# MisEty/X-SLAM

Hardware: AMD Instinct MI355X
Metric: fps XKinectFusion 512^3 TSDF 640x480 CSFD @1/2/4/8 GPU; HBM GB/s on integrate (higher is better)
Workload: dtype f32 (complex<f32> CSFD)

## Files before the change

### include/xslam_amd.h

```cpp
#ifndef XSLAM_AMD_H
#define XSLAM_AMD_H
#include <stddef.h>
#include <stdint.h>

#ifdef __cplusplus
extern "C" {
#endif

const char *xs_last_error(void);

unsigned xs_const_div_prepare(float c);
unsigned xs_const_div_state(float c);
int xs_const_div_enable(int on);
int xs_abi_version(void);

int xs_init_volume(float *value, int *weight, float *grad, size_t step_bytes, const int *res, int z0, int z1, void *stream);

int xs_scale_depth(const uint16_t *depth, size_t depth_step, int rows, int cols, float *scaled, size_t scaled_step, void *stream);
int xs_scale_depth_max(const uint16_t *depth, size_t depth_step, int rows, int cols, float *scaled, size_t scaled_step,
                       float *max_dev, void *stream);
size_t xs_depth_tiles_bytes(int rows, int cols);
int xs_scale_depth_tiles(const uint16_t *depth, size_t depth_step, int rows, int cols, float *scaled, size_t scaled_step,
                         float *max_dev, void *tiles_dev, void *stream);
int xs_depth_tiles(const float *scaled, size_t scaled_step, int rows, int cols, void *tiles_dev, void *stream);
// ... 25 lines not shown
int xs_integrate_list_covers(int rows, int cols, const float *intr4, const int *res, float voxel_size, const float *Rv2c18_list,
                             const float *tv2c6_list, float slack_scale, const float *Rv2c18, const float *tv2c6);
size_t xs_integrate_workspace_bytes(const int *res, int nz);

typedef struct xs_integrate_opts {
    unsigned struct_bytes;
    unsigned flags;
    const void *depth_tiles;
    void *signmap;
    void *start_event, *stop_event;
} xs_integrate_opts;
int xs_integrate_scaled_ex2(const float *depth_scaled, size_t scaled_step, int rows, int cols, const float *intr4, int max_weight,
                            const int *res, float voxel_size, const float *Rv2c18, const float *tv2c6, float tranc_dist, float *value,
                            int *weight, float *grad, size_t vol_step, float threshold, int z0, int z1,
                            unsigned long long *updated_dev, const float *depth_max_dev, void *workspace, const xs_integrate_opts *opts, void *stream);
int xs_integrate_classify_ex(int rows, int cols, const float *intr4, const int *res, float voxel_size, const float *Rv2c18, const float *tv2c6,
                             float tranc_dist, int z0, int z1, const float *depth_max_dev, void *workspace, float slack_scale,
                             const xs_integrate_opts *opts, void *stream);
typedef struct xs_raycast_opts {
    unsigned struct_bytes;
    int signmap_shift;
    const void *signmap;
    float signmap_tranc_dist;
    float *pyr_vmap1, *pyr_nmap1;
    size_t pyr_step1;
    float *pyr_vmap2, *pyr_nmap2;
    size_t pyr_step2;
    void *completion_event;
    int *steps_dev;
    int pyramid_built;
} xs_raycast_opts;
int xs_raycast_ex(const float *intr4, const float *Rc2v18, const float *tc2v6, const float *Rv2w18, const float *tv2w6,
                  float tranc_dist, const int *res, float voxel_size, const float *value, const float *grad, size_t vol_step,
                  float *vmap, float *nmap, size_t map_step, int rows, int cols, unsigned long long *hits_dev, float *workspace,
                  xs_raycast_opts *opts, void *stream);
int xs_raycast_slab_ex(const float *intr4, const float *Rc2v18, const float *tc2v6, const float *Rv2w18, const float *tv2w6,
                       float tranc_dist, const int *res, float voxel_size, const float *value, const float *grad, size_t vol_step,
                       int zs0, int zs1, int z0, int z1, float *vmap, float *nmap, size_t map_step, int rows, int cols, int *keys_dev,
                       const xs_raycast_opts *opts, void *stream);
int xs_resize_pyramid_ex(const float *vmap0, const float *nmap0, size_t in_step, int rows0, int cols0, float *vmap1, float *nmap1,
                         size_t mid_step, float *vmap2, float *nmap2, size_t out_step, void *completion_event, void *stream);

size_t xs_tsdf_reduce_workspace_bytes(void);
int xs_tsdf_reduce_workspace_init(void *workspace, void *stream);
int xs_compute_local_tsdf_hessian(const float *depth_scaled, size_t scaled_step, int rows, int cols, const float *intr4,
                                  const int *res, float voxel_size, const float *Rv2c36, const float *tv2c12, float tranc_dist,
                                  const float *gt, float *real_out, float *grad_out, float *hess_out, int *count_out, int z0, int z1,
                                  void *workspace, double *out4_dev, void *stream);
int xs_compute_local_tsdf_loss(const float *depth_scaled, size_t scaled_step, int rows, int cols, const float *intr4, const int *res,
                               float voxel_size, const float *Rv2c9, const float *tv2c3, float tranc_dist, const float *gt,
                               float *real_out, int *count_out, int z0, int z1, void *workspace, double *out2_dev, void *stream);

int xs_bilateral_filter(const uint16_t *src, size_t src_step, int rows, int cols, float *dst, size_t dst_step, void *stream);
int xs_pyr_down(const float *src, size_t src_step, int src_rows, int src_cols, float *dst, size_t dst_step, void *stream);
int xs_create_vmap(const float *intr4, const float *depth, size_t depth_step, int rows, int cols, float *vmap, size_t vmap_step,
                   void *stream);
int xs_create_nmap(const float *vmap, float *nmap, size_t map_step, int rows, int cols, void *stream);
int xs_create_vnmaps(int levels, const float *intr4s, const float *const *depths, const size_t *depth_steps, int rows0, int cols0,
                     float *const *vmaps, float *const *nmaps, const size_t *map_steps, void *stream);
int xs_create_vnmaps_real(int levels, const float *intr4s, const float *const *depths, const size_t *depth_steps, int rows0, int cols0,
                          float *const *vmaps, float *const *nmaps, const size_t *map_steps, float *const *vreal, float *const *nreal,
                          const size_t *real_steps, void *stream);
int xs_resize_vmap(const float *in, size_t in_step, int src_rows, int src_cols, float *out, size_t out_step, void *stream);
int xs_resize_nmap(const float *in, size_t in_step, int src_rows, int src_cols, float *out, size_t out_step, void *stream);
int xs_resize_pyramid(const float *vmap0, const float *nmap0, size_t in_step, int rows0, int cols0, float *vmap1, float *nmap1,
                      size_t mid_step, float *vmap2, float *nmap2, size_t out_step, void *stream);

int xs_raycast(const float *intr4, const float *Rc2v18, const float *tc2v6, const float *Rv2w18, const float *tv2w6,
               float tranc_dist, const int *res, float voxel_size, const float *value, const float *grad, size_t vol_step,
               float *vmap, float *nmap, size_t map_step, int rows, int cols, unsigned long long *hits_dev, float *workspace,
               void *stream);

int xs_raycast_signmap_shift(const float *intr4, float voxel_size, float tranc_dist);
size_t xs_signmap_bytes(const int *res, int shift);
int xs_signmap_reset(void *signmap, const int *res, int shift, float tranc_dist, void *stream);
int xs_signmap_rebuild(void *signmap, const int *res, int shift, float tranc_dist, const float *value, size_t vol_step, void *stream);
int xs_signmap_rebuild_slab(void *signmap, const int *res, int shift, float tranc_dist, const float *value, size_t vol_step, int zs0, int zs1,
                            void *stream);


int xs_raycast_slab(const float *intr4, const float *Rc2v18, const float *tc2v6, const float *Rv2w18, const float *tv2w6,
                    float tranc_dist, const int *res, float voxel_size, const float *value, const float *grad, size_t vol_step,
                    int zs0, int zs1, int z0, int z1, float *vmap, float *nmap, size_t map_step, int rows, int cols, int *keys_dev,
                    void *stream);
int xs_raycast_compose_mask(const int *own_keys_dev, const int *min_keys_dev, float *vmap, float *nmap, size_t map_step, int rows,
                            int cols, void *stream);
int xs_raycast_compose_finish(const int *min_keys_dev, float *vmap, float *nmap, size_t map_step, int rows, int cols,
                              unsigned long long *hits_dev, void *stream);
size_t xs_raycast_compose_entry_bytes(void);
int xs_raycast_compose_pack(const int *own_keys_dev, const int *min_keys_dev, const float *vmap, const float *nmap, size_t map_step, int rows, int cols,
                            void *entries_dev, int *count_dev, void *stream);
int xs_raycast_compose_scatter(const void *entries_dev, long n, float *vmap, float *nmap, size_t map_step, int rows, int cols, void *stream);

int xs_tsdf_gauss_newton_terms(const float *depth_scaled, size_t scaled_step, int rows, int cols, const float *intr4, const int *res,
                               float voxel_size, const float *Rv2c108, const float *tv2c36, float tranc_dist, const float *gt, int z0, int z1,
                               void *workspace, double *out29_dev, void *stream);
typedef struct xs_gn_opts {
    unsigned struct_bytes;
    unsigned mailbox_seq;
    const void *pose_mailbox;
    double *publish_host;
    unsigned long long publish_seq;
} xs_gn_opts;
int xs_tsdf_gauss_newton_terms_ex(const float *depth_scaled, size_t scaled_step, int rows, int cols, const float *intr4, const int *res,
                                  float voxel_size, const float *Rv2c108, const float *tv2c36, float tranc_dist, const float *gt, int z0, int z1,
                                  void *workspace, double *out29_dev, const xs_gn_opts *opts, void *stream);
// ... 258 lines not shown
```

### x-slam_amd/capi.py

```python
import ctypes as C
import os

import numpy as np

_HERE = os.path.dirname(os.path.abspath(__file__))
LIB_PATH = os.path.join(_HERE, "libxslam_hip.so")

_vp = C.c_void_p
_sz = C.c_size_t
_f32p = C.POINTER(C.c_float)
_i32p = C.POINTER(C.c_int)
_f64p = C.POINTER(C.c_double)


class XsError(RuntimeError):
    pass


def _load():
    if not os.path.exists(LIB_PATH):
        raise ImportError(
            f"{LIB_PATH} not found: build the HIP extension first (python -c 'import __graft_entry__ as g; g.build()' "
            "or make -C x-slam_amd/csrc).  There is no CPU fallback.")
    return C.CDLL(LIB_PATH)
# ... 72 lines not shown
    "xs_frontier_label_bytes": (_sz, [_i32p]),
    "xs_frontier_workspace_bytes": (_sz, [_i32p, C.c_int]),
    "xs_frontier_mask": (C.c_int, [_vp, _i32p, _vp, _vp]),
    "xs_frontier_label": (C.c_int, [_vp, _i32p, C.c_int, _vp, _vp, _i32p, _vp]),
    "xs_frontier_clusters": (C.c_int, [_vp, _vp, _i32p, C.c_int, _vp, _vp, C.POINTER(C.c_uint), _vp, _vp]),
    "xs_frontier_expand": (C.c_int, [_vp, _i32p, _vp, _vp]),
    "xs_integrate_scaled_ex2": (C.c_int, [_vp, _sz, C.c_int, C.c_int, _f32p, C.c_int, _i32p, C.c_float, _f32p, _f32p, C.c_float, _vp, _vp, _vp,
                                         _sz, C.c_float, C.c_int, C.c_int, _vp, _vp, _vp, C.POINTER(IntegrateOpts), _vp]),
    "xs_integrate_classify_ex": (C.c_int, [C.c_int, C.c_int, _f32p, _i32p, C.c_float, _f32p, _f32p, C.c_float, C.c_int, C.c_int, _vp, _vp,
                                           C.c_float, C.POINTER(IntegrateOpts), _vp]),
    "xs_raycast_ex": (C.c_int, [_f32p, _f32p, _f32p, _f32p, _f32p, C.c_float, _i32p, C.c_float, _vp, _vp, _sz, _vp, _vp, _sz,
                                C.c_int, C.c_int, _vp, _vp, C.POINTER(RaycastOpts), _vp]),
    "xs_raycast_slab_ex": (C.c_int, [_f32p, _f32p, _f32p, _f32p, _f32p, C.c_float, _i32p, C.c_float, _vp, _vp, _sz, C.c_int, C.c_int,
                                     C.c_int, C.c_int, _vp, _vp, _sz, C.c_int, C.c_int, _vp, C.POINTER(RaycastOpts), _vp]),
    "xs_resize_pyramid_ex": (C.c_int, [_vp, _vp, _sz, C.c_int, C.c_int, _vp, _vp, _sz, _vp, _vp, _sz, _vp, _vp]),
    "xs_last_error": (C.c_char_p, []),
    "xs_abi_version": (C.c_int, []),
    "xs_init_volume": (C.c_int, [_vp, _vp, _vp, _sz, _i32p, C.c_int, C.c_int, _vp]),
    "xs_scale_depth": (C.c_int, [_vp, _sz, C.c_int, C.c_int, _vp, _sz, _vp]),
    "xs_integrate_tsdf_volume": (C.c_int, [_vp, _sz, C.c_int, C.c_int, _f32p, C.c_int, _i32p, C.c_float, _f32p, _f32p, C.c_float,
                                           _vp, _vp, _vp, _sz, _vp, _sz, C.c_float, C.c_int, C.c_int, _vp, _vp]),
    "xs_integrate_scaled": (C.c_int, [_vp, _sz, C.c_int, C.c_int, _f32p, C.c_int, _i32p, C.c_float, _f32p, _f32p, C.c_float,
                                      _vp, _vp, _vp, _sz, C.c_float, C.c_int, C.c_int, _vp, _vp, _vp, _vp]),
    "xs_integrate_scaled_ex": (C.c_int, [_vp, _sz, C.c_int, C.c_int, _f32p, C.c_int, _i32p, C.c_float, _f32p, _f32p, C.c_float, _vp, _vp, _vp,
                                        _sz, C.c_float, C.c_int, C.c_int, _vp, _vp, _vp, C.c_uint, _vp]),
    "xs_integrate_workspace_clear": (C.c_int, [_vp, _vp]),
    "xs_integrate_fold_counts": (C.c_int, [_vp, _vp, _vp]),
    "xs_integrate_classify": (C.c_int, [C.c_int, C.c_int, _f32p, _i32p, C.c_float, _f32p, _f32p, C.c_float, C.c_int, C.c_int, _vp, _vp,
                                        C.c_float, C.c_uint, _vp]),
    "xs_integrate_list_covers": (C.c_int, [C.c_int, C.c_int, _f32p, _i32p, C.c_float, _f32p, _f32p, C.c_float, _f32p, _f32p]),
    "xs_integrate_workspace_bytes": (_sz, [_i32p, C.c_int]),
    "xs_scale_depth_max": (C.c_int, [_vp, _sz, C.c_int, C.c_int, _vp, _sz, _vp, _vp]),
    "xs_scale_depth_tiles": (C.c_int, [_vp, _sz, C.c_int, C.c_int, _vp, _sz, _vp, _vp, _vp]),
    "xs_depth_tiles": (C.c_int, [_vp, _sz, C.c_int, C.c_int, _vp, _vp]),
    "xs_depth_tiles_bytes": (_sz, [C.c_int, C.c_int]),
    "xs_tsdf_reduce_workspace_bytes": (_sz, []),
    "xs_tsdf_band_segs_bytes": (_sz, [_i32p, C.c_int, C.c_int]),
    "xs_tsdf_band_build": (C.c_int, [_vp, _i32p, C.c_int, C.c_int, C.POINTER(BandIndex), _vp]),
    "xs_tsdf_band_workspace_bytes": (_sz, [C.c_int]),
    "xs_tsdf_gauss_newton_terms_band": (C.c_int, [C.c_int, C.POINTER(_vp), _sz, C.c_int, C.c_int, _f32p, C.c_float, _f32p, _f32p, C.c_float,
                                                  C.POINTER(BandIndex), _vp, _vp, _vp]),
    "xs_tsdf_pose_hessian_workspace_bytes": (_sz, [C.c_int]),
    "xs_tsdf_pose_hessian_band": (C.c_int, [C.c_int, C.POINTER(_vp), _sz, C.c_int, C.c_int, _f32p, C.c_float, _f32p, _f32p, C.c_float,
                                            C.POINTER(BandIndex), _vp, _vp, _vp]),
    "xs_tsdf_score_poses_workspace_bytes": (_sz, [C.c_int]),
    "xs_tsdf_score_poses_band": (C.c_int, [C.c_int, _vp, _sz, C.c_int, C.c_int, _f32p, C.c_float, _f32p, _f32p, C.c_float, C.POINTER(BandIndex), _vp,
                                           _vp, _vp]),
    "xs_tsdf_reduce_workspace_init": (C.c_int, [_vp, _vp]),
    "xs_compute_local_tsdf_hessian": (C.c_int, [_vp, _sz, C.c_int, C.c_int, _f32p, _i32p, C.c_float, _f32p, _f32p, C.c_float, _vp,
                                                _vp, _vp, _vp, _vp, C.c_int, C.c_int, _vp, _vp, _vp]),
    "xs_compute_local_tsdf_loss": (C.c_int, [_vp, _sz, C.c_int, C.c_int, _f32p, _i32p, C.c_float, _f32p, _f32p, C.c_float, _vp,
                                             _vp, _vp, C.c_int, C.c_int, _vp, _vp, _vp]),
    "xs_bilateral_filter": (C.c_int, [_vp, _sz, C.c_int, C.c_int, _vp, _sz, _vp]),
    "xs_pyr_down": (C.c_int, [_vp, _sz, C.c_int, C.c_int, _vp, _sz, _vp]),
    "xs_create_vmap": (C.c_int, [_f32p, _vp, _sz, C.c_int, C.c_int, _vp, _sz, _vp]),
    "xs_create_nmap": (C.c_int, [_vp, _vp, _sz, C.c_int, C.c_int, _vp]),
    "xs_create_vnmaps": (C.c_int, [C.c_int, _f32p, C.POINTER(_vp), C.POINTER(_sz), C.c_int, C.c_int, C.POINTER(_vp), C.POINTER(_vp),
                                   C.POINTER(_sz), _vp]),
    "xs_create_vnmaps_real": (C.c_int, [C.c_int, _f32p, C.POINTER(_vp), C.POINTER(_sz), C.c_int, C.c_int, C.POINTER(_vp), C.POINTER(_vp),
                                        C.POINTER(_sz), C.POINTER(_vp), C.POINTER(_vp), C.POINTER(_sz), _vp]),
    "xs_resize_vmap": (C.c_int, [_vp, _sz, C.c_int, C.c_int, _vp, _sz, _vp]),
    "xs_resize_nmap": (C.c_int, [_vp, _sz, C.c_int, C.c_int, _vp, _sz, _vp]),
    "xs_raycast": (C.c_int, [_f32p, _f32p, _f32p, _f32p, _f32p, C.c_float, _i32p, C.c_float, _vp, _vp, _sz, _vp, _vp, _sz,
                             C.c_int, C.c_int, _vp, _vp, _vp]),
    "xs_raycast_slab": (C.c_int, [_f32p, _f32p, _f32p, _f32p, _f32p, C.c_float, _i32p, C.c_float, _vp, _vp, _sz, C.c_int, C.c_int,
                                  C.c_int, C.c_int, _vp, _vp, _sz, C.c_int, C.c_int, _vp, _vp]),
    "xs_raycast_compose_mask": (C.c_int, [_vp, _vp, _vp, _vp, _sz, C.c_int, C.c_int, _vp]),
    "xs_raycast_compose_finish": (C.c_int, [_vp, _vp, _vp, _sz, C.c_int, C.c_int, _vp, _vp]),
    "xs_raycast_compose_entry_bytes": (_sz, []),
    "xs_raycast_compose_pack": (C.c_int, [_vp, _vp, _vp, _vp, _sz, C.c_int, C.c_int, _vp, _vp, _vp]),
    "xs_raycast_compose_scatter": (C.c_int, [_vp, C.c_long, _vp, _vp, _sz, C.c_int, C.c_int, _vp]),
    "xs_resize_pyramid": (C.c_int, [_vp, _vp, _sz, C.c_int, C.c_int, _vp, _vp, _sz, _vp, _vp, _sz, _vp]),
    "xs_tsdf_gauss_newton_terms": (C.c_int, [_vp, _sz, C.c_int, C.c_int, _f32p, _i32p, C.c_float, _f32p, _f32p, C.c_float, _vp, C.c_int,
                                             C.c_int, _vp, _vp, _vp]),
    "xs_tsdf_gauss_newton_terms_ex": (C.c_int, [_vp, _sz, C.c_int, C.c_int, _f32p, _i32p, C.c_float, _f32p, _f32p, C.c_float, _vp, C.c_int,
                                                C.c_int, _vp, _vp, _vp, _vp]),
    "xs_gn_publish_bytes": (_sz, []),
    "xs_gn_mailbox_bytes": (_sz, []),
    "xs_gn_post_poses": (None, [_vp, _f32p, _f32p, C.c_uint, C.c_int]),
    "xs_gn_publish_sums": (C.c_int, [_vp, C.c_int, _vp, C.c_ulonglong, _vp]),
    "xs_extract_workspace_bytes": (_sz, [_i32p]),
    "xs_extract_points": (C.c_int, [_vp, _sz, _i32p, C.c_float, C.c_int, C.c_int, C.c_int, _vp, _sz, _vp, C.POINTER(_sz), C.POINTER(_sz), _vp]),
    "xs_extract_normals": (C.c_int, [_vp, _sz, _i32p, C.c_float, C.c_int, C.c_int, _vp, _sz, _vp, _vp]),
    "xs_tsdf_merge_workspace_bytes": (_sz, [_i32p, _i32p]),
    "xs_tsdf_diff_workspace_bytes": (_sz, [_i32p, _i32p]),
    "xs_tsdf_diff": (C.c_int, [_vp, _vp, _sz, _i32p, _vp, _vp, _sz, _i32p, _f32p, C.c_int, C.c_float, C.c_float, C.c_uint, _vp, _vp, _vp, _vp, _vp]),
    "xs_tsdf_pack_bricks": (_sz, [_i32p, C.c_int]),
    "xs_tsdf_pack_workspace_bytes": (_sz, [_i32p, C.c_int]),
    "xs_tsdf_pack_classify": (C.c_int, [_vp, _vp, _vp, _sz, _i32p, C.c_int, _vp, _vp, _vp, _vp]),
    "xs_tsdf_pack_offsets": (C.c_int, [_vp, _sz, _vp, _vp, _vp]),
    "xs_tsdf_pack_gather": (C.c_int, [_vp, _vp, _vp, _sz, _i32p, C.c_int, _vp, _vp, _sz, _sz, _vp, _vp]),
    "xs_tsdf_unpack": (C.c_int, [_vp, _vp, _vp, _sz, _i32p, C.c_int, _vp, _vp, _sz, _sz, _vp, _vp]),
    "xs_tsdf_merge": (C.c_int, [_vp, _vp, _vp, _sz, _i32p, C.c_int, C.c_int, _vp, _vp, _vp, _sz, _i32p, _f32p, C.c_int, C.c_int, C.c_uint, _vp, _vp, _vp]),
    "xs_tsdf_reintegrate": (C.c_int, [C.c_int, C.POINTER(ReintegrateOp), _sz, C.c_int, C.c_int, _f32p, C.c_int, _i32p, C.c_float, C.c_float, C.c_float, _vp, _vp, _vp,
                                      _sz, C.c_int, C.c_int, _vp, C.c_uint, _vp]),
    "xs_tsdf_align_workspace_bytes": (_sz, [C.c_int]),
    "xs_tsdf_align_terms": (C.c_int, [C.c_int, C.POINTER(BandIndex), _vp, _vp, _sz, _i32p, _f32p, C.c_int, C.c_float, _vp, _vp, _vp]),
    "xs_tsdf_score_transforms_workspace_bytes": (_sz, [C.c_int]),
    "xs_tsdf_score_transforms": (C.c_int, [C.c_int, C.POINTER(BandIndex), C.c_int, _vp, _vp, _sz, _i32p, _f32p, C.c_int, C.c_float, _vp, _vp, _vp]),
    "xs_tsdf_fuse_accumulator_bytes": (_sz, [_i32p]),
    "xs_tsdf_fuse_points_accumulate": (C.c_int, [C.c_longlong, _vp, _f32p, _f32p, _i32p, C.c_float, C.c_float, C.POINTER(FuseOpts), _vp, _vp, _vp]),
    "xs_tsdf_fuse_points_fold": (C.c_int, [_vp, _vp, _vp, _sz, _i32p, C.c_int, C.c_int, _vp, C.c_int, C.c_int, _vp, _vp]),
    "xs_tsdf_register_workspace_bytes": (_sz, [C.c_int]),
    "xs_tsdf_register_terms": (C.c_int, [C.c_int, C.c_longlong, _vp, _f32p, _vp, _vp, _sz, _i32p, C.c_float, C.c_int, C.c_float, _vp, _vp, _vp]),
    "xs_mesh_workspace_bytes": (_sz, [_i32p, C.POINTER(MeshOpts)]),
    "xs_extract_mesh": (C.c_int, [_vp, _vp, _vp, _sz, _i32p, C.c_float, C.POINTER(MeshOpts), _vp, _vp, _vp, _vp, _sz, _vp, _sz, _vp,
# ... 220 lines not shown
    return _lib.xs_integrate_workspace_bytes(r.ctypes.data_as(_i32p), int(r[2]) if nz is None else nz)


def integrate_listed(workspace):
    import torch
    pair = workspace[:8].view(torch.int32).cpu().numpy()
    return int(pair[0]), int(pair[1])


def integrate_list_layout(res, nz=None):
    r = _ia(res, 3)
    nz = int(r[2]) if nz is None else nz
    cap = -(-int(r[0]) // 32) * -(-int(r[1]) // 8) * -(-nz // 2)
    first = 256 + 8192 * 4
    list_bytes = (first + cap * 4 + 255) // 256 * 256
    class_bytes = (cap * 16 + 255) // 256 * 256
    return first, cap, list_bytes, list_bytes + class_bytes + (1 << 20)


def tsdf_reduce_workspace_init(workspace, stream=None):
    check(_lib.xs_tsdf_reduce_workspace_init(_ptr(workspace), _stream(stream)))


def tsdf_reduce_workspace_bytes():
    return _lib.xs_tsdf_reduce_workspace_bytes()


def compute_local_tsdf_hessian(depth_scaled, scaled_step, rows, cols, intr, res, voxel_size, Rv2c, tv2c, tranc_dist, gt, workspace, out4,
                               volumes=None, z0=0, z1=None, stream=None):
    r = _ia(res, 3)
    k, R, t = _fa(intr, 4), _fa(Rv2c, 36), _fa(tv2c, 12)
    z1 = int(r[2]) if z1 is None else z1
    vols = [_ptr(v) for v in volumes] if volumes else [None] * 4
    check(_lib.xs_compute_local_tsdf_hessian(_ptr(depth_scaled), scaled_step, rows, cols, k.ctypes.data_as(_f32p), r.ctypes.data_as(_i32p),
                                             voxel_size, R.ctypes.data_as(_f32p), t.ctypes.data_as(_f32p), tranc_dist, _ptr(gt), vols[0],
                                             vols[1], vols[2], vols[3], z0, z1, _ptr(workspace), _ptr(out4), _stream(stream)))


def compute_local_tsdf_loss(depth_scaled, scaled_step, rows, cols, intr, res, voxel_size, Rv2c, tv2c, tranc_dist, gt, workspace, out2,
                            volumes=None, z0=0, z1=None, stream=None):
    r = _ia(res, 3)
    k, R, t = _fa(intr, 4), _fa(Rv2c, 9), _fa(tv2c, 3)
    z1 = int(r[2]) if z1 is None else z1
    vols = [_ptr(v) for v in volumes] if volumes else [None] * 2
    check(_lib.xs_compute_local_tsdf_loss(_ptr(depth_scaled), scaled_step, rows, cols, k.ctypes.data_as(_f32p), r.ctypes.data_as(_i32p),
                                          voxel_size, R.ctypes.data_as(_f32p), t.ctypes.data_as(_f32p), tranc_dist, _ptr(gt), vols[0],
                                          vols[1], z0, z1, _ptr(workspace), _ptr(out2), _stream(stream)))


def bilateral_filter(src, src_step, rows, cols, dst, dst_step, stream=None):
    check(_lib.xs_bilateral_filter(_ptr(src), src_step, rows, cols, _ptr(dst), dst_step, _stream(stream)))


def pyr_down(src, src_step, src_rows, src_cols, dst, dst_step, stream=None):
    check(_lib.xs_pyr_down(_ptr(src), src_step, src_rows, src_cols, _ptr(dst), dst_step, _stream(stream)))


def create_vmap(intr, depth, depth_step, rows, cols, vmap, vmap_step, stream=None):
    k = _fa(intr, 4)
    check(_lib.xs_create_vmap(k.ctypes.data_as(_f32p), _ptr(depth), depth_step, rows, cols, _ptr(vmap), vmap_step, _stream(stream)))


def create_vnmaps(intrs, depths, depth_steps, rows0, cols0, vmaps, nmaps, map_steps, stream=None, vreal=None, nreal=None, real_steps=None):
    n = len(depths)
    k = np.ascontiguousarray(intrs, dtype=np.float32).reshape(-1)
    assert k.size == 4 * n
    P = lambda ts: (_vp * n)(*[_ptr(t) for t in ts])
    S = lambda xs: (_sz * n)(*[int(x) for x in xs])
    if vreal is None:
        check(_lib.xs_create_vnmaps(n, k.ctypes.data_as(_f32p), P(depths), S(depth_steps), rows0, cols0, P(vmaps), P(nmaps), S(map_steps),
                                    _stream(stream)))
    else:
        check(_lib.xs_create_vnmaps_real(n, k.ctypes.data_as(_f32p), P(depths), S(depth_steps), rows0, cols0, P(vmaps), P(nmaps), S(map_steps),
                                         P(vreal), P(nreal), S(real_steps), _stream(stream)))


def tsdf_gauss_newton_terms(depth_scaled, scaled_step, rows, cols, intr, res, voxel_size, Rv2c6, tv2c6, tranc_dist, gt, workspace, out29,
                            z0=0, z1=None, stream=None):
    r = _ia(res, 3)
    k, R, t = _fa(intr, 4), _fa(Rv2c6, 108), _fa(tv2c6, 36)
    z1 = int(r[2]) if z1 is None else z1
    check(_lib.xs_tsdf_gauss_newton_terms(_ptr(depth_scaled), scaled_step, rows, cols, k.ctypes.data_as(_f32p), r.ctypes.data_as(_i32p),
                                          voxel_size, R.ctypes.data_as(_f32p), t.ctypes.data_as(_f32p), tranc_dist, _ptr(gt), z0, z1,
                                          _ptr(workspace), _ptr(out29), _stream(stream)))


BAND_OVER_CAPACITY = -3
BAND_MAX_FRAMES = 32


def tsdf_band_segs_bytes(res, z0=0, z1=None):
    r = _ia(res, 3)
    return int(_lib.xs_tsdf_band_segs_bytes(r.ctypes.data_as(_i32p), z0, int(r[2]) if z1 is None else z1))


def tsdf_band_build_raw(gt, res, z0, z1, keys, values, capacity, segs, stream=None):
    r = _ia(res, 3)
    idx = BandIndex()
    idx.keys, idx.values, idx.capacity, idx.segs = _ptr(keys), _ptr(values), int(capacity), _ptr(segs)
    rc = _lib.xs_tsdf_band_build(_ptr(gt), r.ctypes.data_as(_i32p), z0, z1, C.byref(idx), _stream(stream))
    if rc != BAND_OVER_CAPACITY:
        check(rc)
    return rc, idx


def tsdf_band_build(gt, res, z0=0, z1=None, stream=None):
# ... 857 lines not shown
```

### x-slam_amd/csrc/xs_map.hip

```cpp
#include <hip/hip_ext.h>
#include "xs_device.h"
#include "../../include/xslam_amd.h"

using namespace xs;

namespace {
constexpr float kSigmaColor = 30.f;
constexpr float kSigmaSpace = 4.5f;
constexpr int BR = 6, BD = 2 * BR + 1;
constexpr int BTX = 64, BTY = 4;
}

namespace {
constexpr int TP = 4;
typedef float f32x2 __attribute__((ext_vector_type(2)));
constexpr float kSkip = -1048576.f;
constexpr float kSpaceInvHalf = 0.5f / (kSigmaSpace * kSigmaSpace);
constexpr float kColorInvHalf = 0.5f / (kSigmaColor * kSigmaColor);
constexpr int TW = BTX + 2 * BR, TH = BTY + 2 * BR;
constexpr int NTAPS = BD * BD;
constexpr int clamp_tap(int tap) { return tap < NTAPS ? tap : 0; }
constexpr int tap_offset(int tap) { return (clamp_tap(tap) / BD) * TW + clamp_tap(tap) % BD; }
constexpr float space_term(int tap) {
    const int dx = clamp_tap(tap) % BD - BR, dy = clamp_tap(tap) / BD - BR;
    return (float)(dx * dx + dy * dy) * kSpaceInvHalf;
}
}

__global__ void __launch_bounds__(BTX *BTY) k_bilateral(const uint16_t *src, size_t sstep, int rows, int cols, cfloat *dst, size_t dstep) {
    __shared__ float tile[TH][TW];
    const int bx = blockIdx.x * BTX, by = blockIdx.y * BTY;
    const int tid = threadIdx.y * BTX + threadIdx.x;
    for (int i = tid; i < TH * TW; i += BTX * BTY) {
        int ty = i / TW, tx = i % TW;
        int gy = by + ty - BR, gx = bx + tx - BR;
        float v = kSkip;
        if (gy >= 0 && gy < rows - 1 && gx >= 0 && gx < cols - 1) v = (float)row_ptr(src, sstep, gy)[gx];
        tile[ty][tx] = v;
    }
    __syncthreads();
    const int x = bx + threadIdx.x, y = by + threadIdx.y;
    if (x >= cols || y >= rows) return;
    const f32x2 value = f32x2((float)row_ptr(src, sstep, y)[x]);
    const float *win = &tile[threadIdx.y][threadIdx.x];
    float sum1 = 0, sum2 = 0;
#pragma unroll
    for (int g = 0; g < NTAPS; g += 2 * TP) {
        f32x2 tmp[TP], p[TP], ph[TP], pl[TP], e[TP], w[TP], tw[TP];
#pragma unroll
        for (int k = 0; k < TP; ++k) tmp[k] = f32x2{win[tap_offset(g + 2 * k)], win[tap_offset(g + 2 * k + 1)]};
#pragma unroll
        for (int k = 0; k < TP; ++k) p[k] = value - tmp[k];
#pragma unroll
        for (int k = 0; k < TP; ++k) p[k] = p[k] * p[k];
#pragma unroll
        for (int k = 0; k < TP; ++k) p[k] = f32x2{space_term(g + 2 * k), space_term(g + 2 * k + 1)} + p[k] * kColorInvHalf;
#pragma unroll
        for (int k = 0; k < TP; ++k) ph[k] = p[k] * -0x1.715476p+0f;
#pragma unroll
        for (int k = 0; k < TP; ++k) pl[k] = __builtin_elementwise_fma(p[k], f32x2(-0x1.715476p+0f), -ph[k]);
#pragma unroll
        for (int k = 0; k < TP; ++k) pl[k] = __builtin_elementwise_fma(p[k], f32x2(-0x1.4ae0bep-26f), pl[k]);
#pragma unroll
        for (int k = 0; k < TP; ++k) e[k] = __builtin_elementwise_rint(ph[k]);
#pragma unroll
        for (int k = 0; k < TP; ++k) ph[k] = (ph[k] - e[k]) + pl[k];
#pragma unroll
        for (int k = 0; k < TP; ++k)
            w[k] = f32x2{__builtin_ldexpf(__builtin_amdgcn_exp2f(ph[k].x), (int)e[k].x), __builtin_ldexpf(__builtin_amdgcn_exp2f(ph[k].y), (int)e[k].y)};
#pragma unroll
        for (int k = 0; k < TP; ++k) tw[k] = tmp[k] * w[k];
#pragma unroll
        for (int k = 0; k < TP; ++k) {
            if (g + 2 * k < NTAPS) { sum1 += tw[k].x; sum2 += w[k].x; asm("" : "+v"(sum1)); }
            if (g + 2 * k + 1 < NTAPS) { sum1 += tw[k].y; sum2 += w[k].y; asm("" : "+v"(sum1)); }
        }
    }
    int round = __float2int_rn(sum1 / sum2);
    if (round > 5000 || round < 200) round = 0;
    round = max(0, min(round, 32767));
    row_ptr(dst, dstep, y)[x] = cfloat(__int2float_rd(round), 0.f);
}

extern "C" int xs_bilateral_filter(const uint16_t *src, size_t src_step, int rows, int cols, float *dst, size_t dst_step, void *stream) {
    if (!src || !dst) return xs_set_error(hipErrorInvalidValue, "xs_bilateral_filter: null pointer");
    if (rows <= 0 || cols <= 0) return 0;
    dim3 block(BTX, BTY), grid(div_up(cols, BTX), div_up(rows, BTY));
    hipLaunchKernelGGL(k_bilateral, grid, block, 0, (hipStream_t)stream, src, src_step, rows, cols, (cfloat *)dst, dst_step);
    XS_CHECK(hipGetLastError());
    return 0;
}

__global__ void __launch_bounds__(256) k_pyr_down(const cfloat *src, size_t sstep, int srows, int scols, cfloat *dst, size_t dstep,
                                                  int drows, int dcols, float sigma_color) {
    const int x = blockIdx.x * blockDim.x + threadIdx.x;
    const int y = blockIdx.y * blockDim.y + threadIdx.y;
    if (x >= dcols || y >= drows) return;
    const int D = 5;
    const int center = __float2int_rn(row_ptr(src, sstep, 2 * y)[2 * x].re);
    const int tx = min(2 * x - D / 2 + D, scols - 1);
    const int ty = min(2 * y - D / 2 + D, srows - 1);
    int sum = 0, count = 0;
    for (int cy = max(0, 2 * y - D / 2); cy < ty; ++cy)
        for (int cx = max(0, 2 * x - D / 2); cx < tx; ++cx) {
            const int val = __float2int_rn(row_ptr(src, sstep, cy)[cx].re);
            if (abs(val - center) < 3 * sigma_color) { sum += val; ++count; }
        }
    row_ptr(dst, dstep, y)[x] = cfloat(__int2float_rd(sum / count), 0.f);
}

extern "C" int xs_pyr_down(const float *src, size_t src_step, int src_rows, int src_cols, float *dst, size_t dst_step, void *stream) {
    if (!src || !dst) return xs_set_error(hipErrorInvalidValue, "xs_pyr_down: null pointer");
    int drows = src_rows / 2, dcols = src_cols / 2;
    if (drows <= 0 || dcols <= 0) return 0;
    dim3 block(64, 4), grid(div_up(dcols, 64), div_up(drows, 4));
    hipLaunchKernelGGL(k_pyr_down, grid, block, 0, (hipStream_t)stream, (const cfloat *)src, src_step, src_rows, src_cols, (cfloat *)dst,
                       dst_step, drows, dcols, kSigmaColor);
    XS_CHECK(hipGetLastError());
    return 0;
}

__global__ void __launch_bounds__(256) k_vmap(const cfloat *depth, size_t dstep, int rows, int cols, cfloat *vmap, size_t mstep, float fx_inv,
                                              float fy_inv, float cx, float cy) {
    const int u = threadIdx.x + blockIdx.x * blockDim.x;
    const int v = threadIdx.y + blockIdx.y * blockDim.y;
    if (u >= cols || v >= rows) return;
    cfloat z = row_ptr(depth, dstep, v)[u];
    z /= 1000.f;
    if (z.re != 0) {
        const cfloat vx = z * (float(u) - cx) * fx_inv;
        const cfloat vy = z * (float(v) - cy) * fy_inv;
        row_ptr(vmap, mstep, v)[u] = vx;
        row_ptr(vmap, mstep, v + rows)[u] = vy;
        row_ptr(vmap, mstep, v + rows * 2)[u] = z;
    } else
        row_ptr(vmap, mstep, v)[u] = cfloat(qnan_f(), 0.f);
}

extern "C" int xs_create_vmap(const float *intr4, const float *depth, size_t depth_step, int rows, int cols, float *vmap, size_t vmap_step,
                              void *stream) {
    if (!intr4 || !depth || !vmap) return xs_set_error(hipErrorInvalidValue, "xs_create_vmap: null pointer");
// ... 205 lines not shown
```

Measured before the change: 4144.

## Replace per-tap bilateral exp with LDS lookup table indexed by radius and depth difference

The bilateral filter now precomputes exact weights for every distinct squared radius and integer depth difference (up to 433, beyond which the weight is zero) into a device table. Each block copies the table to LDS and looks weights up using v_sad_u32 on pre-scaled depths. Each thread handles two pixels per window load, and the block height is chosen from the CU count. This removes the exp2/ldexp arithmetic per tap at the cost of LDS table loads, a one-time build kernel with per-device event sync, and larger LDS use that may limit occupancy. The old path is kept as a direct variant, and a check kernel is added to verify the table matches the direct weights bit for bit.

Result: slower. 4068 (-1.8%).

```diff
diff --git a/include/xslam_amd.h b/include/xslam_amd.h
--- a/include/xslam_amd.h
+++ b/include/xslam_amd.h
@@ -101,6 +101,8 @@
                                float *real_out, int *count_out, int z0, int z1, void *workspace, double *out2_dev, void *stream);
 
 int xs_bilateral_filter(const uint16_t *src, size_t src_step, int rows, int cols, float *dst, size_t dst_step, void *stream);
+int xs_bilateral_filter_direct(const uint16_t *src, size_t src_step, int rows, int cols, float *dst, size_t dst_step, void *stream);
+int xs_bilateral_table_check(int d_table_last, int d_last, unsigned *report, void *stream);
 int xs_pyr_down(const float *src, size_t src_step, int src_rows, int src_cols, float *dst, size_t dst_step, void *stream);
 int xs_create_vmap(const float *intr4, const float *depth, size_t depth_step, int rows, int cols, float *vmap, size_t vmap_step,
                    void *stream);
diff --git a/x-slam_amd/capi.py b/x-slam_amd/capi.py
--- a/x-slam_amd/capi.py
+++ b/x-slam_amd/capi.py
@@ -148,6 +148,8 @@
     "xs_compute_local_tsdf_loss": (C.c_int, [_vp, _sz, C.c_int, C.c_int, _f32p, _i32p, C.c_float, _f32p, _f32p, C.c_float, _vp,
                                              _vp, _vp, C.c_int, C.c_int, _vp, _vp, _vp]),
     "xs_bilateral_filter": (C.c_int, [_vp, _sz, C.c_int, C.c_int, _vp, _sz, _vp]),
+    "xs_bilateral_filter_direct": (C.c_int, [_vp, _sz, C.c_int, C.c_int, _vp, _sz, _vp]),
+    "xs_bilateral_table_check": (C.c_int, [C.c_int, C.c_int, _vp, _vp]),
     "xs_pyr_down": (C.c_int, [_vp, _sz, C.c_int, C.c_int, _vp, _sz, _vp]),
     "xs_create_vmap": (C.c_int, [_f32p, _vp, _sz, C.c_int, C.c_int, _vp, _sz, _vp]),
     "xs_create_nmap": (C.c_int, [_vp, _vp, _sz, C.c_int, C.c_int, _vp]),
@@ -474,6 +476,14 @@
     check(_lib.xs_bilateral_filter(_ptr(src), src_step, rows, cols, _ptr(dst), dst_step, _stream(stream)))
 
 
+def bilateral_filter_direct(src, src_step, rows, cols, dst, dst_step, stream=None):
+    check(_lib.xs_bilateral_filter_direct(_ptr(src), src_step, rows, cols, _ptr(dst), dst_step, _stream(stream)))
+
+
+def bilateral_table_check(d_table_last, d_last, report, stream=None):
+    check(_lib.xs_bilateral_table_check(d_table_last, d_last, _ptr(report), _stream(stream)))
+
+
 def pyr_down(src, src_step, src_rows, src_cols, dst, dst_step, stream=None):
     check(_lib.xs_pyr_down(_ptr(src), src_step, src_rows, src_cols, _ptr(dst), dst_step, _stream(stream)))
 
diff --git a/x-slam_amd/csrc/xs_map.hip b/x-slam_amd/csrc/xs_map.hip
--- a/x-slam_amd/csrc/xs_map.hip
+++ b/x-slam_amd/csrc/xs_map.hip
@@ -11,23 +11,136 @@
 constexpr int BTX = 64, BTY = 4;
 }
 
+#include <mutex>
+#include <utility>
 namespace {
-constexpr int TP = 4;
-typedef float f32x2 __attribute__((ext_vector_type(2)));
 constexpr float kSkip = -1048576.f;
 constexpr float kSpaceInvHalf = 0.5f / (kSigmaSpace * kSigmaSpace);
 constexpr float kColorInvHalf = 0.5f / (kSigmaColor * kSigmaColor);
+constexpr int NTAPS = BD * BD;
+constexpr int tap_dx(int tap) { return tap % BD - BR; }
+constexpr int tap_dy(int tap) { return tap / BD - BR; }
+__host__ __device__ constexpr float space_of_r2(int r2) { return (float)r2 * kSpaceInvHalf; }
+
+constexpr int kRows = 27;
+constexpr int kR2[kRows] = {0, 1, 2, 4, 5, 8, 9, 10, 13, 16, 17, 18, 20, 25, 26, 29, 32, 34, 36, 37, 40, 41, 45, 50, 52, 61, 72};
+constexpr int row_of_r2(int r2) {
+    for (int i = 0; i < kRows; ++i)
+        if (kR2[i] == r2) return i;
+    return -1;
+}
+constexpr int row_of_tap(int tap) { return row_of_r2(tap_dx(tap) * tap_dx(tap) + tap_dy(tap) * tap_dy(tap)); }
+constexpr bool every_tap_has_a_row() {
+    for (int tap = 0; tap < NTAPS; ++tap)
+        if (row_of_tap(tap) < 0) return false;
+    return true;
+}
+static_assert(every_tap_has_a_row(), "kR2 misses a dx^2 + dy^2 of the window");
+constexpr int kDMax = 433;
+constexpr int kRowLen = kDMax + 1;
+constexpr int kTableFloats = (kRows * kRowLen + 3) / 4 * 4;
+
+__device__ __forceinline__ float bilateral_weight(float space, float d) {
+    float p = d * d;
+    p = p * kColorInvHalf;
+    p = space + p;
+    const float ph = p * -0x1.715476p+0f;
+    float pl = __builtin_fmaf(p, -0x1.715476p+0f, -ph);
+    pl = __builtin_fmaf(p, -0x1.4ae0bep-26f, pl);
+    const float e = __builtin_rintf(ph);
+    const float frac = (ph - e) + pl;
+    return __builtin_ldexpf(__builtin_amdgcn_exp2f(frac), (int)e);
+}
+
+__device__ __attribute__((aligned(16))) float g_bilateral_table[kTableFloats];
+}
+
+__global__ void __launch_bounds__(256) k_bilateral_build_table() {
+    const int i = blockIdx.x * 256 + threadIdx.x;
+    if (i >= kTableFloats) return;
+    const int row = i / kRowLen, d = i % kRowLen;
+    g_bilateral_table[i] = row < kRows ? bilateral_weight(space_of_r2(kR2[row]), (float)d) : 0.f;
+}
+
+namespace {
+constexpr int TBX = 128, TBY_MAX = 16, TBY_MIN = 4;
+constexpr int TTW = TBX + 2 * BR, TTH_MAX = TBY_MAX + 2 * BR;
+constexpr unsigned kPad4 = 4u * (65535u + 1048576u);
+static_assert(kPad4 < (1u << 24), "the padding tap converts to float exactly");
+static_assert(sizeof(float) * kTableFloats + sizeof(unsigned) * TTW * TTH_MAX <= 64 * 1024, "static LDS of k_bilateral");
+
+struct BilateralSums { float sum1 = 0, sum2 = 0; };
+__device__ __forceinline__ void table_tap(const float *tab_row, unsigned v4, unsigned tap4, float tap, BilateralSums &s) {
+    unsigned off;
+    asm("v_sad_u32 %0, %1, %2, 0" : "=v"(off) : "v"(v4), "v"(tap4));
+    off = min(off, 4u * kDMax);
+    const float w = *(const float *)((const char *)tab_row + off);
+    const float tw = tap * w;
+    s.sum1 += tw;
+    s.sum2 += w;
+    asm("" : "+v"(s.sum1), "+v"(s.sum2));
+}
+template <int DY, int... DX>
+__device__ __forceinline__ void table_row(std::integer_sequence<int, DX...>, const unsigned *win, const float *tab, unsigned v4a, unsigned v4b,
+                                          BilateralSums &a, BilateralSums &b) {
+    unsigned e[BD + 1];
+    float f[BD + 1];
+#pragma unroll
+    for (int j = 0; j < BD + 1; j += 2) {
+        const uint2 c = *(const uint2 *)&win[DY * TTW + j];
+        e[j] = c.x; e[j + 1] = c.y;
+    }
+#pragma unroll
+    for (int j = 0; j < BD + 1; ++j) f[j] = (float)e[j] * 0.25f;
+    (table_tap(tab + row_of_tap(DY * BD + DX) * kRowLen, v4a, e[DX], f[DX], a), ...);
+    (table_tap(tab + row_of_tap(DY * BD + DX) * kRowLen, v4b, e[DX + 1], f[DX + 1], b), ...);
+}
+template <int... DY>
+__device__ __forceinline__ void table_window(std::integer_sequence<int, DY...>, const unsigned *win, const float *tab, unsigned v4a, unsigned v4b,
+                                             BilateralSums &a, BilateralSums &b) {
+    (table_row<DY>(std::make_integer_sequence<int, BD>(), win, tab, v4a, v4b, a, b), ...);
+}
+
+__device__ __forceinline__ cfloat bilateral_result(float sum1, float sum2) {
+    int round = __float2int_rn(sum1 / sum2);
+    if (round > 5000 || round < 200) round = 0;
+    round = max(0, min(round, 32767));
+    return cfloat(__int2float_rd(round), 0.f);
+}
+}
+
+__global__ void __launch_bounds__(64 * TBY_MAX) k_bilateral(const uint16_t *src, size_t sstep, int rows, int cols, cfloat *dst, size_t dstep) {
+    __shared__ __attribute__((aligned(16))) float tab[kTableFloats];
+    __shared__ __attribute__((aligned(8))) unsigned tile[TTH_MAX][TTW];
+    const int brows = blockDim.y, nthreads = 64 * brows;
+    const int bx = blockIdx.x * TBX, by = blockIdx.y * brows;
+    const int tid = threadIdx.y * 64 + threadIdx.x;
+    for (int i = tid; i < kTableFloats / 4; i += nthreads) ((float4 *)tab)[i] = ((const float4 *)g_bilateral_table)[i];
+    for (int i = tid; i < (brows + 2 * BR) * TTW; i += nthreads) {
+        int ty = i / TTW, tx = i % TTW;
+        int gy = by + ty - BR, gx = bx + tx - BR;
+        unsigned v = kPad4;
+        if (gy >= 0 && gy < rows - 1 && gx >= 0 && gx < cols - 1) v = 4u * row_ptr(src, sstep, gy)[gx];
+        tile[ty][tx] = v;
+    }
+    __syncthreads();
+    const int x = bx + 2 * threadIdx.x, y = by + threadIdx.y;
+    if (x >= cols || y >= rows) return;
+    const bool right = x + 1 < cols;
+    const uint16_t *srow = row_ptr(src, sstep, y);
+    const unsigned v4a = 4u * srow[x], v4b = right ? 4u * srow[x + 1] : 0u;
+    BilateralSums a, b;
+    table_window(std::make_integer_sequence<int, BD>(), &tile[threadIdx.y][2 * threadIdx.x], tab, v4a, v4b, a, b);
+    cfloat *drow = row_ptr(dst, dstep, y);
+    drow[x] = bilateral_result(a.sum1, a.sum2);
+    if (right) drow[x + 1] = bilateral_result(b.sum1, b.sum2);
+}
+
+namespace {
 constexpr int TW = BTX + 2 * BR, TH = BTY + 2 * BR;
-constexpr int NTAPS = BD * BD;
-constexpr int clamp_tap(int tap) { return tap < NTAPS ? tap : 0; }
-constexpr int tap_offset(int tap) { return (clamp_tap(tap) / BD) * TW + clamp_tap(tap) % BD; }
-constexpr float space_term(int tap) {
-    const int dx = clamp_tap(tap) % BD - BR, dy = clamp_tap(tap) / BD - BR;
-    return (float)(dx * dx + dy * dy) * kSpaceInvHalf;
-}
-}
-
-__global__ void __launch_bounds__(BTX *BTY) k_bilateral(const uint16_t *src, size_t sstep, int rows, int cols, cfloat *dst, size_t dstep) {
+}
+
+__global__ void __launch_bounds__(BTX *BTY) k_bilateral_direct(const uint16_t *src, size_t sstep, int rows, int cols, cfloat *dst, size_t dstep) {
     __shared__ float tile[TH][TW];
     const int bx = blockIdx.x * BTX, by = blockIdx.y * BTY;
     const int tid = threadIdx.y * BTX + threadIdx.x;
@@ -41,52 +154,95 @@
     __syncthreads();
     const int x = bx + threadIdx.x, y = by + threadIdx.y;
     if (x >= cols || y >= rows) return;
-    const f32x2 value = f32x2((float)row_ptr(src, sstep, y)[x]);
+    const float value = (float)row_ptr(src, sstep, y)[x];
     const float *win = &tile[threadIdx.y][threadIdx.x];
     float sum1 = 0, sum2 = 0;
 #pragma unroll
-    for (int g = 0; g < NTAPS; g += 2 * TP) {
-        f32x2 tmp[TP], p[TP], ph[TP], pl[TP], e[TP], w[TP], tw[TP];
-#pragma unroll
-        for (int k = 0; k < TP; ++k) tmp[k] = f32x2{win[tap_offset(g + 2 * k)], win[tap_offset(g + 2 * k + 1)]};
-#pragma unroll
-        for (int k = 0; k < TP; ++k) p[k] = value - tmp[k];
-#pragma unroll
-        for (int k = 0; k < TP; ++k) p[k] = p[k] * p[k];
-#pragma unroll
-        for (int k = 0; k < TP; ++k) p[k] = f32x2{space_term(g + 2 * k), space_term(g + 2 * k + 1)} + p[k] * kColorInvHalf;
-#pragma unroll
-        for (int k = 0; k < TP; ++k) ph[k] = p[k] * -0x1.715476p+0f;
-#pragma unroll
-        for (int k = 0; k < TP; ++k) pl[k] = __builtin_elementwise_fma(p[k], f32x2(-0x1.715476p+0f), -ph[k]);
-#pragma unroll
-        for (int k = 0; k < TP; ++k) pl[k] = __builtin_elementwise_fma(p[k], f32x2(-0x1.4ae0bep-26f), pl[k]);
-#pragma unroll
-        for (int k = 0; k < TP; ++k) e[k] = __builtin_elementwise_rint(ph[k]);
-#pragma unroll
-        for (int k = 0; k < TP; ++k) ph[k] = (ph[k] - e[k]) + pl[k];
-#pragma unroll
-        for (int k = 0; k < TP; ++k)
-            w[k] = f32x2{__builtin_ldexpf(__builtin_amdgcn_exp2f(ph[k].x), (int)e[k].x), __builtin_ldexpf(__builtin_amdgcn_exp2f(ph[k].y), (int)e[k].y)};
-#pragma unroll
-        for (int k = 0; k < TP; ++k) tw[k] = tmp[k] * w[k];
-#pragma unroll
-        for (int k = 0; k < TP; ++k) {
-            if (g + 2 * k < NTAPS) { sum1 += tw[k].x; sum2 += w[k].x; asm("" : "+v"(sum1)); }
-            if (g + 2 * k + 1 < NTAPS) { sum1 += tw[k].y; sum2 += w[k].y; asm("" : "+v"(sum1)); }
-        }
-    }
-    int round = __float2int_rn(sum1 / sum2);
-    if (round > 5000 || round < 200) round = 0;
-    round = max(0, min(round, 32767));
-    row_ptr(dst, dstep, y)[x] = cfloat(__int2float_rd(round), 0.f);
+    for (int tap = 0; tap < NTAPS; ++tap) {
+        const float tmp = win[(tap / BD) * TW + tap % BD];
+        const float w = bilateral_weight(space_of_r2(tap_dx(tap) * tap_dx(tap) + tap_dy(tap) * tap_dy(tap)), value - tmp);
+        const float tw = tmp * w;
+        sum1 += tw;
+        sum2 += w;
+    }
+    row_ptr(dst, dstep, y)[x] = bilateral_result(sum1, sum2);
+}
+
+namespace {
+constexpr int kMaxDevices = 64;
+struct TableState { std::mutex mu; bool launched = false; hipStream_t stream = nullptr; hipEvent_t built = nullptr; int cus = 0; };
+TableState g_table_state[kMaxDevices];
+}
+static int bilateral_table_ready(hipStream_t stream, int *cus) {
+    int dev = 0;
+    XS_CHECK(hipGetDevice(&dev));
+    if (dev < 0 || dev >= kMaxDevices) return xs_set_error(hipErrorInvalidDevice, "xs_bilateral_filter: device ordinal beyond the table states");
+    TableState &t = g_table_state[dev];
+    std::lock_guard<std::mutex> lk(t.mu);
+    if (!t.launched) {
+        XS_CHECK(hipDeviceGetAttribute(&t.cus, hipDeviceAttributeMultiprocessorCount, dev));
+        XS_CHECK(hipEventCreateWithFlags(&t.built, hipEventDisableTiming));
+        hipLaunchKernelGGL(k_bilateral_build_table, dim3(div_up(kTableFloats, 256)), dim3(256), 0, stream);
+        XS_CHECK(hipGetLastError());
+        XS_CHECK(hipEventRecord(t.built, stream));
+        t.stream = stream;
+        t.launched = true;
+    } else if (stream != t.stream)
+        XS_CHECK(hipStreamWaitEvent(stream, t.built, 0));
+    if (cus) *cus = t.cus;
+    return 0;
+}
+static int bilateral_block_rows(int rows, int cols, int cus) {
+    int best = TBY_MIN, best_share = 0;
+    for (int r = TBY_MIN; r <= TBY_MAX; ++r) {
+        const int share = div_up(div_up(cols, TBX) * div_up(rows, r), cus > 0 ? cus : 1) * div_up(r, 4);
+        if (r == TBY_MIN || share <= best_share) { best = r; best_share = share; }
+    }
+    return best;
 }
 
 extern "C" int xs_bilateral_filter(const uint16_t *src, size_t src_step, int rows, int cols, float *dst, size_t dst_step, void *stream) {
     if (!src || !dst) return xs_set_error(hipErrorInvalidValue, "xs_bilateral_filter: null pointer");
     if (rows <= 0 || cols <= 0) return 0;
+    int cus = 0;
+    if (int rc = bilateral_table_ready((hipStream_t)stream, &cus)) return rc;
+    const int brows = bilateral_block_rows(rows, cols, cus);
+    dim3 block(64, brows), grid(div_up(cols, TBX), div_up(rows, brows));
+    hipLaunchKernelGGL(k_bilateral, grid, block, 0, (hipStream_t)stream, src, src_step, rows, cols, (cfloat *)dst, dst_step);
+    XS_CHECK(hipGetLastError());
+    return 0;
+}
+extern "C" int xs_bilateral_filter_direct(const uint16_t *src, size_t src_step, int rows, int cols, float *dst, size_t dst_step, void *stream) {
+    if (!src || !dst) return xs_set_error(hipErrorInvalidValue, "xs_bilateral_filter_direct: null pointer");
+    if (rows <= 0 || cols <= 0) return 0;
     dim3 block(BTX, BTY), grid(div_up(cols, BTX), div_up(rows, BTY));
-    hipLaunchKernelGGL(k_bilateral, grid, block, 0, (hipStream_t)stream, src, src_step, rows, cols, (cfloat *)dst, dst_step);
+    hipLaunchKernelGGL(k_bilateral_direct, grid, block, 0, (hipStream_t)stream, src, src_step, rows, cols, (cfloat *)dst, dst_step);
+    XS_CHECK(hipGetLastError());
+    return 0;
+}
+
+__global__ void __launch_bounds__(256) k_bilateral_table_check(int d_table_last, int d_last, unsigned *report) {
+    const int d = blockIdx.x * 256 + threadIdx.x;
+    if (d > d_last) return;
+    if (d <= d_table_last) {
+        unsigned bad = 0;
+        for (int row = 0; row < kRows; ++row)
+            bad += __float_as_uint(g_bilateral_table[row * kRowLen + min(d, kDMax)]) != __float_as_uint(bilateral_weight(space_of_r2(kR2[row]), (float)d));
+        if (bad) atomicAdd(&report[0], bad);
+    }
+    const unsigned w0 = __float_as_uint(bilateral_weight(space_of_r2(0), (float)d));
+    if (w0 != 0) {
+        if (d >= kDMax) atomicAdd(&report[1], 1u);
+        atomicMax(&report[2], (unsigned)d + 1u);
+    }
+    if (d < kRows && __float_as_uint(g_bilateral_table[d * kRowLen + kDMax]) != 0) atomicAdd(&report[3], 1u);
+    if (d == 0) { report[4] = kDMax; report[5] = kRows; }
+}
+extern "C" int xs_bilateral_table_check(int d_table_last, int d_last, unsigned *report, void *stream) {
+    if (!report || d_table_last < 0 || d_last < d_table_last) return xs_set_error(hipErrorInvalidValue, "xs_bilateral_table_check: bad arguments");
+    if (int rc = bilateral_table_ready((hipStream_t)stream, nullptr)) return rc;
+    XS_CHECK(hipMemsetAsync(report, 0, 8 * sizeof(unsigned), (hipStream_t)stream));
+    hipLaunchKernelGGL(k_bilateral_table_check, dim3(div_up(d_last + 1, 256)), dim3(256), 0, (hipStream_t)stream, d_table_last, d_last, report);
     XS_CHECK(hipGetLastError());
     return 0;
 }
```
